# google/zopfli

Measured on AMD Instinct MI355X. Metric: input MB/s at numiterations=15 (gzip, bit-exact vs reference), higher is better.
Workload: dtype u8 (f32/f64 cost DP); 1 GPU; class-T synthetic (text-like, the enwik8 stand-in) 100000000 B per GPU, numiterations=15, blocksplitting=0, gzip, BASELINE configs[1]; total_bytes=100000000, master_blocks=100, gather=none (one rank)

## Files before the change

include/zopfli_amd.h:

```cpp
#ifndef ZOPFLI_AMD_H_
#define ZOPFLI_AMD_H_

#include <stddef.h>
#include <stdint.h>

#ifdef __cplusplus
extern "C" {
#endif

#if defined(__GNUC__)
#pragma GCC visibility push(default)
#endif



typedef struct ZopfliOptions {
  int verbose;
  int verbose_more;
  int numiterations;
  int blocksplitting;
  int blocksplittinglast;
  int blocksplittingmax;
} ZopfliOptions;

// ... 172 lines not shown
int zmx_last_host_timing(double* out2);

int zmx_last_match_timing(double* out4);
int zmx_last_match_walk(double* out3);

typedef void (*zmx_oom_hook_t)(int device);
void zmx_set_oom_hook(zmx_oom_hook_t hook);
int zmx_ctx_set_share(zmx_ctx* ctx, unsigned contexts_on_device);
int zmx_ctx_trim_cache(zmx_ctx* ctx);
int zmx_ctx_set_priority(zmx_ctx* ctx, int level);

int zmx_set_match_kernel(int kernel);

int zmx_last_seg_stats(double* out8);

#if defined(__GNUC__)
#pragma GCC visibility pop
#endif

#ifdef __cplusplus
}
#endif

#endif
```

zopfli_amd/api.py:

```python
import ctypes
import os

from ._build import LIB

if os.environ.get("ZOPFLI_AMD_LIB"):
    LIB = os.environ["ZOPFLI_AMD_LIB"]

FORMAT_GZIP, FORMAT_ZLIB, FORMAT_DEFLATE = 0, 1, 2
CRC32, ADLER32 = 0, 1
ZMX_HIST = 320


class ZopfliOptions(ctypes.Structure):
    _fields_ = [("verbose", ctypes.c_int), ("verbose_more", ctypes.c_int), ("numiterations", ctypes.c_int),
                ("blocksplitting", ctypes.c_int), ("blocksplittinglast", ctypes.c_int),
                ("blocksplittingmax", ctypes.c_int)]

    def __init__(self, numiterations=15, blocksplitting=1, blocksplittingmax=15, verbose=0, verbose_more=0):
        super().__init__(verbose, verbose_more, numiterations, blocksplitting, 0, blocksplittingmax)


class ZmxBlock(ctypes.Structure):
    _fields_ = [("instart", ctypes.c_uint64), ("inend", ctypes.c_uint64)]

# ... 63 lines not shown
                                    P(ctypes.c_uint32), P(ctypes.c_uint32)]
    lib.zmx_store_download.argtypes = [vp, vp, sz, ctypes.c_int, P(ctypes.c_uint16), P(ctypes.c_uint16), sz]
    lib.zmx_find_longest_match.argtypes = [vp, vp, sz, sz, P(ctypes.c_uint16), P(ctypes.c_uint16),
                                           P(ctypes.c_uint16)]
    lib.zmx_length_array_download.argtypes = [vp, vp, sz, P(ctypes.c_uint16)]
    lib.zmx_hash_links_download.argtypes = [vp, vp, sz, P(ctypes.c_uint16), P(ctypes.c_uint16), P(ctypes.c_uint16)]
    lib.zmx_deflate_range.argtypes = [vp, opt, sz, sz, ctypes.c_int, P(_u8p), P(sz)]
    lib.zmx_checksum.argtypes = [vp, ctypes.c_int, sz, sz, P(ctypes.c_uint32)]
    lib.zmx_checksum_combine.argtypes = [ctypes.c_int, ctypes.c_uint32, ctypes.c_uint32, ctypes.c_uint64]
    lib.zmx_checksum_combine.restype = ctypes.c_uint32
    lib.zmx_chunks_merge.argtypes = [P(vp), P(sz), sz, P(ctypes.c_ubyte), P(_u8p), P(sz)]
    lib.zmx_last_timing.argtypes = [P(ctypes.c_double)]
    lib.zmx_last_kernel_timing.argtypes = [P(ctypes.c_double)]
    lib.zmx_last_host_timing.argtypes = [P(ctypes.c_double)]
    lib.zmx_last_seg_stats.argtypes = [P(ctypes.c_double)]
    lib.zmx_last_match_timing.argtypes = [P(ctypes.c_double)]
    lib.zmx_set_match_kernel.argtypes = [ctypes.c_int]
    lib.zmx_dist_unique_id.argtypes = [ctypes.c_char_p]
    lib.zmx_dist_init.argtypes = [vp, ctypes.c_int, ctypes.c_int, ctypes.c_char_p, P(vp)]
    lib.zmx_dist_destroy.argtypes = [vp]
    lib.zmx_dist_destroy.restype = None
    lib.zmx_dist_comm_count.argtypes = [vp]
    lib.zmx_dist_gather.argtypes = [vp, vp, sz, P(vp), P(sz)]
    lib.zmx_set_kernel_timing.argtypes = [ctypes.c_int]
    lib.zmx_set_kernel_timing.restype = None
    lib.zmx_set_kernel_timing(1)
    return lib


def library(path=None):
# ... 73 lines not shown
    m = (ctypes.c_double * 4)()
    lib.zmx_last_match_timing(m)
    d["match_kernel"], d["hash_kernels"], d["table_builds"], d["positions_matched"] = m[0], m[1], m[2], m[3]
    w = (ctypes.c_double * 3)()
    lib.zmx_last_match_walk(w)
    d["skip_walk_lane_iterations"], d["skip_walk_wave_iterations"], d["skip_walk_positions"] = w[0], w[1], w[2]
    return d


def last_seg_stats(lib=None):
    lib = lib or library()
    t = (ctypes.c_double * 8)()
    lib.zmx_last_seg_stats(t)
    keys = ["tasks", "accepted", "rerun_state", "rerun_level", "rerun_tie", "positions_rerun", "rerun_values", "positions"]
    return dict(zip(keys, list(t)))


class Context:

    def __init__(self, device=0, lib=None):
        self.lib = lib or library()
        self.handle = ctypes.c_void_p()
        self._input = None
        self._segments = None
        if self.lib.zmx_ctx_create(device, ctypes.byref(self.handle)) != 0:
            raise RuntimeError("zmx_ctx_create: " + self.error())

    def error(self):
        return (self.lib.zmx_last_error() or b"").decode()

# ... 326 lines not shown
```

zopfli_amd/csrc/device/zmx_hip.hip:

```cpp
#include <hip/hip_runtime.h>

#include <algorithm>
#include <atomic>
#include <cmath>
#include <cstdio>
#include <cstdlib>
#include <cstring>
#include <mutex>
#include <string>
#include <unordered_map>
#include <vector>

#include "zmx_kernels.h"
#include "zmx_match2.h"
#ifdef ZMX_EXPERIMENTS
#include "zmx_match3.h"
#include "zmx_match4.h"
#else
#define BK_CH 32768u
#endif
#include "zmx_match5.h"
#include "zmx_dp4.h"
#include "zmx_dp5.h"
#include "zmx_encode.h"
// ... 4 lines not shown
#include "zmx_png_brute.h"
#include "zmx_blockcost.h"
#include "zopfli_amd.h"
#include "../host/symbol_check.h"
#include "../host/thread_pool.h"

namespace {

thread_local std::string g_err;
struct ThreadStats {
  double kernel_seconds[3];
  double squeeze_launches;
  double match5[3];
  double match[4];
  double seg[8];
};
static_assert(sizeof(ThreadStats) == 19 * sizeof(double), "zmx_internal_stats_take / _add move 19 doubles");
thread_local ThreadStats g_ts = {};
#define g_kernel_seconds g_ts.kernel_seconds
#define g_squeeze_launches g_ts.squeeze_launches
#define g_match5_stats g_ts.match5
#define g_match_stats g_ts.match
#define g_seg_stats g_ts.seg

thread_local bool g_last_oom = false;
thread_local int g_err_class = ZMX_ERR_NONE;

int Fail(const char* what, hipError_t e, const char* file, int line) {
  char buf[512];
  std::snprintf(buf, sizeof(buf), "%s: %s (%s:%d)", what, hipGetErrorString(e), file, line);
  g_err = buf;
  g_last_oom = e == hipErrorOutOfMemory;
  g_err_class = g_last_oom ? ZMX_ERR_OUT_OF_MEMORY : ZMX_ERR_DEVICE;
  if (g_last_oom) (void)hipGetLastError();
  return -1;
}
int FailMsg(const std::string& m) {
  g_err = m;
// ... 110 lines not shown
  double* d_cost = nullptr;
  double* d_mincost = nullptr;
  int* d_slot = nullptr;
  uint2* d_dph = nullptr;
  u64* d_block_edges = nullptr;
  u32* d_badpos = nullptr;
  size_t badpos_words = 0;
  bool badpos_clean = false;
  u64* d_code_base = nullptr;
  u16* d_codes = nullptr;
  double* d_wtab = nullptr;
  u32* d_badcodes = nullptr;
  u32* d_seg_off = nullptr;
  u32* d_extab = nullptr;
  uint2* d_seginfo = nullptr;
  std::vector<u32> seg_off;
  std::vector<u64> block_edges;
  std::vector<u32> tile_off;
  u32* d_counters = nullptr;
  u32* d_flags = nullptr;
  unsigned char* d_runin = nullptr;
  unsigned char* d_runout = nullptr;
  unsigned char* h_runin = nullptr;
  unsigned char* h_runout = nullptr;
  size_t h_runin_cap = 0, h_runout_cap = 0;
  size_t runin_bytes = 0, runout_bytes = 0;
  u64* d_prof = nullptr;
  std::vector<SegTask> tasks;
  std::vector<u32> task_off;
  SegTask* d_tasks = nullptr;
// ... 268 lines not shown
  if (kernel != 0 && kernel != 2 && kernel != 5) return FailMsg("zmx_set_match_kernel: 0, 2 or 5");
#endif
  g_match_kernel.store(kernel, std::memory_order_relaxed);
  return 0;
}

size_t zmx_internal_input_size(zmx_ctx* ctx) { return ctx->insize; }
int zmx_internal_device(zmx_ctx* ctx) { return ctx->device; }
void zmx_internal_set_error(const char* msg) { g_err = msg; g_err_class = ZMX_ERR_DEVICE; }
void zmx_internal_set_error_class(const char* msg, int cls) { g_err = msg; g_err_class = cls; }
const unsigned char* zmx_internal_input_host(zmx_ctx* ctx) { return ctx->h_in; }

void zmx_internal_seg_stats(double* out8, int reset) {
  for (int i = 0; i < 8; ++i) out8[i] = g_seg_stats[i];
  if (reset) for (int i = 0; i < 8; ++i) g_seg_stats[i] = 0;
}

void zmx_internal_match5_stats(double* out3, int reset) {
  for (int i = 0; i < 3; ++i) out3[i] = g_match5_stats[i];
  if (reset) for (int i = 0; i < 3; ++i) g_match5_stats[i] = 0;
}

void zmx_internal_match_stats(double* out4, int reset) {
  for (int i = 0; i < 4; ++i) out4[i] = g_match_stats[i];
  if (reset) for (int i = 0; i < 4; ++i) g_match_stats[i] = 0;
}

void zmx_internal_kernel_stats(double* seconds3, double* squeeze_launches, int reset) {
  for (int i = 0; i < 3; ++i) seconds3[i] = g_kernel_seconds[i];
  *squeeze_launches = g_squeeze_launches;
  if (reset) {
    g_kernel_seconds[0] = g_kernel_seconds[1] = g_kernel_seconds[2] = 0;
    g_squeeze_launches = 0;
  }
}

void zmx_internal_stats_take(double* out19) {
  std::memcpy(out19, &g_ts, sizeof(g_ts));
  g_ts = ThreadStats{};
}
void zmx_internal_stats_add(const double* in19) {
  double* d = reinterpret_cast<double*>(&g_ts);
  for (int i = 0; i < 19; ++i) d[i] += in19[i];
}

static hipError_t PinnedTake(zmx_ctx* c, unsigned char** p, size_t bytes, size_t* cap) {
  size_t best = c->pinned_free.size();
  for (size_t i = 0; i < c->pinned_free.size(); ++i) {
    const size_t k = c->pinned_free[i].second;
    if (k >= bytes && k <= 4 * bytes + 4096 && (best == c->pinned_free.size() || k < c->pinned_free[best].second)) best = i;
  }
  if (best != c->pinned_free.size()) {
    *p = c->pinned_free[best].first;
    *cap = c->pinned_free[best].second;
    c->pinned_free.erase(c->pinned_free.begin() + static_cast<long>(best));
    return hipSuccess;
  }
  *cap = bytes < 4096 ? 4096 : bytes;
// ... 21 lines not shown
  c->device = device;
  HIPCHK(hipStreamCreate(&c->stream));
  for (int i = 0; i < 4; ++i) HIPCHK(hipEventCreate(&c->ev[i]));
  HIPCHK(hipStreamCreate(&c->stream2));
  for (int i = 0; i < 2; ++i) HIPCHK(hipEventCreateWithFlags(&c->ev2[i], hipEventDisableTiming));
  {
    size_t mem_free = 0, mem_total = 0;
    HIPCHK(hipMemGetInfo(&mem_free, &mem_total));
    c->keep_base = std::min<size_t>(kPoolKeepMax, mem_free / 3);
    c->pool_keep = c->keep_base;
    c->code_budget = c->keep_base;
  }

  HIPCHK(hipFuncSetAttribute(reinterpret_cast<const void*>(k_chain), hipFuncAttributeMaxDynamicSharedMemorySize,
                             CH_LDS_BYTES));
#ifdef ZMX_EXPERIMENTS
  HIPCHK(hipFuncSetAttribute(reinterpret_cast<const void*>(k_bucket), hipFuncAttributeMaxDynamicSharedMemorySize,
                             BK_LDS_BYTES));
#endif
  *out = c;
  return 0;
}

int zmx_ctx_set_priority(zmx_ctx* c, int level) {
  DeviceGuard dev_guard(c->device);
  HIPCHK(dev_guard.err);
  const int k = level > 0 ? 1 : level < 0 ? 2 : 0;
  if (!c->alt_stream[0][0]) { c->alt_stream[0][0] = c->stream; c->alt_stream[0][1] = c->stream2; }
  if (k && !c->alt_stream[k][1]) {
    int least = 0, greatest = 0;
// ... 70 lines not shown
  rel(t->d_ssame);
  rel(t->d_chunk_base);
  rel(t->d_recs);
  rel(t->d_pool);
  rel(t->d_la);
  rel(t->d_dph);
  rel(t->d_block_edges);
  rel(t->d_badpos);
  rel(t->d_code_base);
  rel(t->d_codes);
  rel(t->d_wtab);
  rel(t->d_badcodes);
  rel(t->d_seg_off);
  rel(t->d_extab);
  rel(t->d_seginfo);
  rel(t->d_counters);
  rel(t->d_prof);
  rel(t->d_tasks);
  rel(t->d_task_off);
  rel(t->d_wg_tasks);
  rel(t->d_task_kind);
  rel(t->d_run_list);
  rel(t->d_wmeta);
  rel(t->d_runin);
  rel(t->d_runout);
  rel(t->d_winroff);
  rel(t->d_winflag);
  rel(t->d_win_off);
  rel(t->d_lvl);
  rel(t->d_entry);
// ... 151 lines not shown
  } else
#endif
  {
    HIPCHK(PoolAlloc(c, &t->d_links, reg_off));
  }
  HIPCHK(PoolAlloc(c, &t->d_recs, pos_off * 8));
  HIPCHK(PoolAlloc(c, &t->d_la, la_off));
  HIPCHK(PoolAlloc(c, &t->d_store[0], pos_off));
  HIPCHK(PoolAlloc(c, &t->d_store[1], pos_off));
  {
    const size_t in_cost = 0, in_min = in_cost + nb * ZMX_HIST * sizeof(double), in_info = in_min + nb * sizeof(double),
                 in_slot = in_info + 3 * nb * sizeof(float);
    t->runin_bytes = in_slot + nb * sizeof(int);
    const size_t out_hist = 0, out_nsym = out_hist + nb * ZMX_HIST * sizeof(u32), out_stats = out_nsym + nb * sizeof(u32),
                 out_flags = out_stats + 8 * sizeof(u32);
    t->runout_bytes = out_flags + 4 * sizeof(u32);
    HIPCHK(PoolAlloc(c, &t->d_runin, t->runin_bytes));
    HIPCHK(PoolAlloc(c, &t->d_runout, t->runout_bytes));
    HIPCHK(PinnedTake(c, &t->h_runin, t->runin_bytes, &t->h_runin_cap));
    HIPCHK(PinnedTake(c, &t->h_runout, t->runout_bytes, &t->h_runout_cap));
    t->d_cost = reinterpret_cast<double*>(t->d_runin + in_cost);
    t->d_mincost = reinterpret_cast<double*>(t->d_runin + in_min);
    t->d_runinfo = reinterpret_cast<float*>(t->d_runin + in_info);
    t->d_slot = reinterpret_cast<int*>(t->d_runin + in_slot);
    t->d_hist = reinterpret_cast<u32*>(t->d_runout + out_hist);
    t->d_nsym = reinterpret_cast<u32*>(t->d_runout + out_nsym);
    t->d_segstats = reinterpret_cast<u32*>(t->d_runout + out_stats);
    t->d_flags = reinterpret_cast<u32*>(t->d_runout + out_flags);
    HIPCHK(hipMemsetAsync(t->d_segstats, 0, 12 * sizeof(u32), c->stream));
  }
  HIPCHK(PoolAlloc(c, &t->d_dph, pos_off));
  HIPCHK(PoolAlloc(c, &t->d_block_edges, nb));
  t->badpos_words = pos_off / 32 + 4;
  HIPCHK(PoolAlloc(c, &t->d_badpos, t->badpos_words));
  HIPCHK(PoolAlloc(c, &t->d_code_base, nb));
  HIPCHK(PoolAlloc(c, &t->d_wtab, nb * ZMX_WTAB));
  HIPCHK(PoolAlloc(c, &t->d_badcodes, nb * 40));
  HIPCHK(PoolAlloc(c, &t->d_counters, 48));
  HIPCHK(hipMemcpyAsync(t->d_blocks, t->blocks.data(), nb * sizeof(BlockDesc), hipMemcpyHostToDevice, c->stream));
  HIPCHK(hipMemcpyAsync(t->d_tile_off, tile_off.data(), (nb + 1) * sizeof(u32), hipMemcpyHostToDevice, c->stream));
  HIPCHK(hipMemsetAsync(t->d_flags, 0, 4 * sizeof(u32), c->stream));

  HIPCHK(hipEventRecord(c->ev[0], c->stream));
  PoolScope hash_tmp(c);
  u16* d_lev = nullptr;
  u16* d_tot2 = nullptr;
  u16* d_rank2 = nullptr;
  uint4* d_xrec = nullptr;
  u32* d_tot12 = nullptr;
  unsigned long long* d_energy = nullptr;
  u32* d_cmax = nullptr;
  bool skip_any = false, skip_all = false;
  double skip_positions = 0;
  unsigned long long* d_m5stats = nullptr;
  bool join_stream2 = false;
  auto launch_hash = [&](const u64* d_link_lo) -> int {
    if (max_l == 0) return 0;
    const dim3 g1(static_cast<unsigned>((max_l + 256 * SAME_CH - 1) / (256 * SAME_CH)), static_cast<unsigned>(nb));
    hipLaunchKernelGGL(k_same, g1, dim3(256), 0, c->stream, c->d_in, t->d_blocks, t->d_same16, d_link_lo);
    KCHK(c, "k_same");
    HIPCHK(hipGetLastError());
    const dim3 g2(static_cast<unsigned>((max_l + CH_EMIT - 1) / CH_EMIT), static_cast<unsigned>(nb), 2);
#ifdef ZMX_EXPERIMENTS
    if (t->buckets) {
      BucketParams kp;
      kp.in = c->d_in;
      kp.blocks = t->d_blocks;
      kp.same16 = t->d_same16;
      kp.chunk_base = t->d_chunk_base;
      kp.link_lo = d_link_lo;
      for (int h = 0; h < 2; ++h) { kp.sorted[h] = t->d_sorted[h]; kp.rank[h] = t->d_rank[h]; kp.bucket[h] = t->d_bucket[h]; }
      kp.ssame = t->d_ssame;
      hipLaunchKernelGGL(k_bucket, g2, dim3(BK_THREADS), BK_LDS_BYTES, c->stream, kp);
      KCHK(c, "k_bucket");
    } else
#endif
    {
      hipLaunchKernelGGL(k_chain, g2, dim3(64), CH_LDS_BYTES, c->stream, c->d_in, t->d_blocks, t->d_same16, t->d_links, d_link_lo);
      KCHK(c, "k_chain");
      if ((mk == 5 || mk == 0) && d_link_lo == nullptr) {
        skip_any = mk == 5;
        if (mk == 5) for (size_t b = 0; b < nb; ++b) skip_positions += static_cast<double>(t->blocks[b].inend - t->blocks[b].instart);
        const unsigned hits_chunks = static_cast<unsigned>((max_l + RK_CH - 1) / RK_CH);
        {
          static const bool rank_all = [] { const char* e = std::getenv("ZOPFLI_AMD_RANK_ALL"); return e && std::atoi(e) != 0; }();
          if (!d_energy) HIPCHK(hash_tmp.AllocT(&d_energy, nb, "d_energy"));
          if (!d_cmax && !rank_all) HIPCHK(hash_tmp.AllocT(&d_cmax, nb * static_cast<size_t>(hits_chunks) + 1, "d_cmax"));
          HIPCHK(hipMemsetAsync(d_energy, 0, nb * sizeof(unsigned long long), c->stream));
          if (d_cmax) HIPCHK(hipMemsetAsync(d_cmax, 0, (nb * static_cast<size_t>(hits_chunks) + 1) * sizeof(u32), c->stream));
          HitsParams hp;
          hp.in = c->d_in;
          hp.blocks = t->d_blocks;
          hp.same16 = t->d_same16;
          hp.energy = d_energy;
// ... 481 lines not shown
      if (ntk) HIPCHK(hipMemcpyAsync(t->d_task_kind, kind.data(), ntk * sizeof(u32), hipMemcpyHostToDevice, c->stream));
      if (!runs.empty()) HIPCHK(hipMemcpyAsync(t->d_run_list, runs.data(), runs.size() * sizeof(u32), hipMemcpyHostToDevice, c->stream));
      HIPCHK(hipStreamSynchronize(c->stream));
    }
    wg.insert(wg.end(), wg_runs.begin(), wg_runs.end());
    HIPCHK(PoolAlloc(c, &t->d_wg_tasks, wg.size() + 4));
    if (!wg.empty()) HIPCHK(hipMemcpyAsync(t->d_wg_tasks, wg.data(), wg.size() * sizeof(u32), hipMemcpyHostToDevice, c->stream));
    HIPCHK(hipStreamSynchronize(c->stream));
  }
  }
  t->seg_off.assign(nb + 1, 0);
  for (size_t b = 0; b < nb; ++b) t->seg_off[b + 1] = t->seg_off[b] + (t->bsize[b] + TS_SEG - 1) / TS_SEG;
  HIPCHK(PoolAlloc(c, &t->d_seg_off, nb + 1));
  HIPCHK(PoolAlloc(c, &t->d_extab, static_cast<size_t>(t->seg_off[nb]) * GS_STATES));
  HIPCHK(PoolAlloc(c, &t->d_seginfo, t->seg_off[nb]));
  HIPCHK(hipMemcpyAsync(t->d_seg_off, t->seg_off.data(), (nb + 1) * sizeof(u32), hipMemcpyHostToDevice, c->stream));
  HIPCHK(hipStreamSynchronize(c->stream));
  return 0;
}

int zmx_tables_build(zmx_ctx* c, const zmx_block* blocks, size_t nblocks, zmx_tables** out) {
  return zmx_tables_build_from(c, nullptr, blocks, nblocks, out);
}

int zmx_tables_build_matches(zmx_ctx* c, const zmx_block* blocks, size_t nblocks, zmx_tables** out) {
  DeviceGuard dev_guard(c->device);
  HIPCHK(dev_guard.err);
  zmx_tables* t = new zmx_tables();
  g_last_oom = false;
  const int rc = BuildTables(c, blocks, nblocks, t, nullptr, false);
// ... 230 lines not shown
  tp.seg_off = t->d_seg_off;
  tp.nb_total = static_cast<u32>(nb);
  tp.recs = t->d_recs;
  tp.pool = t->d_pool;
  tp.la = t->d_la;
  tp.slot = t->d_slot;
  tp.store0 = t->d_store[0];
  tp.store1 = t->d_store[1];
  tp.hist_out = t->d_hist;
  tp.nsym_out = t->d_nsym;
  tp.flags = t->d_flags;
  tp.extab = t->d_extab;
  tp.seginfo = t->d_seginfo;
  tp.block0 = 0;
  tp.seg0 = 0;
  double ksec[3] = {0, 0, 0};
  const bool timing = KernelTiming();
  const dim3 dpdim(64 * (D3_NB + 2));
  {
    const unsigned nblk = static_cast<unsigned>(nb);
    const unsigned tiles = t->tile_off[nb];
    const unsigned ntask = t->task_off[nb];
    if (timing) HIPCHK(hipEventRecord(c->ev[0], c->stream));
    hipLaunchKernelGGL(k_wtab, dim3(nblk), dim3(256), 0, c->stream, wp);
    KCHK(c, "k_wtab");
    if (tiles && scan_bad) hipLaunchKernelGGL(k_badscan, dim3(tiles), dim3(256), 0, c->stream, bp);
    KCHK(c, "k_badscan");
    HIPCHK(hipGetLastError());
    if (timing) HIPCHK(hipEventRecord(c->ev[1], c->stream));
    {
// ... 46 lines not shown
        } else {
          if (cp.prof) hipLaunchKernelGGL((k_dp5_spec<true, 4, false>), dim3(cap), dim3(64 * D5_WG), 0, c->stream, c2);
          else hipLaunchKernelGGL((k_dp5_spec<false, 4, false>), dim3(cap), dim3(64 * D5_WG), 0, c->stream, c2);
        }
        KCHK(c, "k_dp5_spec");
        hipLaunchKernelGGL(k_dpcheck, dim3(ntask), dim3(64), 0, c->stream, cp);
        KCHK(c, "k_dpcheck");
      }
      if (cp.prof) hipLaunchKernelGGL(k_dp4_fix<true>, dim3(nblk), dpdim, 0, c->stream, cp);
      else hipLaunchKernelGGL(k_dp4_fix<false>, dim3(nblk), dpdim, 0, c->stream, cp);
      KCHK(c, "k_dp4_fix");
    }
    HIPCHK(hipGetLastError());
    if (timing) HIPCHK(hipEventRecord(c->ev[2], c->stream));
    const unsigned nseg = t->seg_off[nb];
    if (nseg) hipLaunchKernelGGL(k_trace_exits, dim3(nseg), dim3(TS_THREADS), 0, c->stream, tp);
    KCHK(c, "k_trace_exits");
    hipLaunchKernelGGL(k_trace_link, dim3(nblk), dim3(64), 0, c->stream, tp);
    KCHK(c, "k_trace_link");
    if (nseg) hipLaunchKernelGGL(k_trace_emit, dim3(nseg), dim3(64), 0, c->stream, tp);
    KCHK(c, "k_trace_emit");
    HIPCHK(hipGetLastError());
    if (timing) HIPCHK(hipEventRecord(c->ev[3], c->stream));
  }
  u32 segstats[8];
  HIPCHK(hipMemcpyAsync(t->h_runout, t->d_runout, t->runout_bytes, hipMemcpyDeviceToHost, c->stream));
  HIPCHK(hipStreamSynchronize(c->stream));
  for (int i = 0; i < 3 && timing; ++i) {
    float ms = 0;
    HIPCHK(hipEventElapsedTime(&ms, c->ev[i], c->ev[i + 1]));
    ksec[i] += ms * 1e-3;
  }
  {
    const u32* o_hist = reinterpret_cast<const u32*>(t->h_runout);
    const u32* o_nsym = o_hist + nb * ZMX_HIST;
    const u32* o_stats = o_nsym + nb;
    const u32* o_flags = o_stats + 8;
    std::memcpy(hist, o_hist, nb * ZMX_HIST * sizeof(u32));
    std::memcpy(nsym, o_nsym, nb * sizeof(u32));
    std::memcpy(segstats, o_stats, sizeof(segstats));
    if (o_flags[1]) {
      char buf[128];
      std::snprintf(buf, sizeof(buf), "zmx_squeeze_run: device consistency flags 0x%x", o_flags[1]);
      return FailFault(buf);
    }
  }
  t->h_hist.assign(hist, hist + nb * ZMX_HIST);
  t->have_hist = true;
  ++t->squeeze_runs;
  {
    for (int i = 0; i < 3; ++i) g_kernel_seconds[i] += ksec[i];
    g_squeeze_launches += 1;
// ... 817 lines not shown
```

zopfli_amd/csrc/device/zmx_kernels.h:

```cpp
#pragma once
#include <hip/hip_runtime.h>
#include <stdint.h>

typedef unsigned char u8;
typedef unsigned short u16;
typedef unsigned int u32;
typedef unsigned long long u64;

struct BlockDesc {
  u64 instart, inend, ws;
  u64 pos_off;
  u64 reg_off;
  u64 la_off;
};

#define ZMX_WINDOW 32768u
#define ZMX_MAX_MATCH 258u
#define ZMX_MAX_CHAIN_HITS 8192
#define ZMX_NONE16 0xffffu

__device__ __forceinline__ int dev_dist_symbol(u32 d) {
  if (d < 5) return (int)d - 1;
  const int l = 31 - __clz((int)(d - 1));
  return 2 * l + (int)(((d - 1) >> (l - 1)) & 1);
// ... 170 lines not shown
      u32 d;
      if (lower) d = lane - (63u - (u32)__clzll((long long)lower));
      else d = old == ZMX_NONE16 ? 0u : r - old;
      if (d > 32767u) d = 0;
      wave_lds_sync();
      if (act && (grp & gt_mask) == 0) head[key] = (u16)r;
      wave_lds_sync();
      const u64 k = t0 + i;
      if (act && k >= e0) {
        if (chain == 0) {
          lk[k].x = (u16)d;
          lk[k].z = sames[i];
        } else {
          lk[k].y = (u16)d;
        }
      }
    }
    __syncthreads();
  }
}

#define MT 2048u
#define MWIN_BYTES (32768u + MT + 288u)
#define SCRATCH_CPS 256u
#define M_XCD_GROUP 16u
#define MATCH_BATCH 8u

struct MatchParams {
  const u8* in;
  const BlockDesc* blocks;
// ... 384 lines not shown
```

zopfli_amd/csrc/device/zmx_trace.h:

```cpp
#pragma once

#define TS_SEG 4096u
#define TS_ENT 258u

struct TraceSegParams {
  const BlockDesc* blocks;
  const u32* seg_off;
  u32 nb_total;
  u32 block0;
  u32 seg0;
  const u32* recs;
  const u32* pool;
  const u16* la;
  const int* slot;
  u32* store0;
  u32* store1;
  u32* hist_out;
  u32* nsym_out;
  u32* flags;
  u32* extab;
  uint2* seginfo;
};

__device__ __forceinline__ void ts_bounds(u32 B, u32 s, u32& lo, u32& hi) {
  hi = B - s * TS_SEG;
  lo = hi > TS_SEG ? hi - TS_SEG : 0u;
}

__device__ __forceinline__ u32 ts_find_block(const u32* seg_off, u32 nb, u32 seg) {
  u32 lo = 0, hi = nb;
  while (hi - lo > 1) {
    const u32 mid = (lo + hi) >> 1;
    if (seg_off[mid] <= seg) lo = mid; else hi = mid;
  }
  return lo;
}

#define TS_ROUNDS 6
#define TS_THREADS 512u

__global__ __launch_bounds__(TS_THREADS) void k_trace_exits(TraceSegParams P) {
  __shared__ u32 s_j[TS_SEG + 1];
  const u32 seg = P.seg0 + blockIdx.x;
  const u32 b = ts_find_block(P.seg_off, P.nb_total, seg);
  const BlockDesc bd = P.blocks[b];
  const u32 B = (u32)(bd.inend - bd.instart);
  u32 lo, hi;
  ts_bounds(B, seg - P.seg_off[b], lo, hi);
  const u16* la = P.la + bd.la_off;
  const u32 n = hi - lo;
  for (u32 x = threadIdx.x + 1; x <= n; x += TS_THREADS) {
    const u32 h = lo + x;
    u32 len = la[h];
    if (len == 0) len = 1;
    if (len > h) len = h;
    const u32 t = h - len;
    s_j[x] = (t > lo ? t - lo : 0x8000u | (lo - t)) | (1u << 16);
  }
// ... 13 lines not shown
    u32 v = s_j[n - j];
    while (!(v & 0x8000u)) {
      const u32 w = s_j[v & 0xffffu];
      v = (w & 0xffffu) | ((v & 0xffff0000u) + (w & 0xffff0000u));
    }
    P.extab[(u64)seg * TS_ENT + j] = (v & 0x7fffu) | (v & 0xffff0000u);
  }
}

__global__ __launch_bounds__(64) void k_trace_link(TraceSegParams P) {
  const u32 b = P.block0 + blockIdx.x;
  const BlockDesc bd = P.blocks[b];
  const u32 B = (u32)(bd.inend - bd.instart);
  const u32 lane = threadIdx.x;
  for (u32 i = lane; i < 320; i += 64) P.hist_out[(u64)b * 320 + i] = 0;
  if (lane != 0) return;
  const u32 s0 = P.seg_off[b], ns = P.seg_off[b + 1] - s0;
  u32 j = 0, off = 0;
  for (u32 s = 0; s < ns; ++s) {
    P.seginfo[s0 + s] = make_uint2(j, off);
    u32 lo, hi;
    ts_bounds(B, s, lo, hi);
    if (hi - lo <= j) {
      P.seginfo[s0 + s] = make_uint2(0xffffffffu, off);
      continue;
    }
    const u32 v = P.extab[(u64)(s0 + s) * TS_ENT + j];
    off += v >> 16;
    j = v & 0xffffu;
  }
  P.nsym_out[b] = off;
}
// ... 137 lines not shown
```

zopfli_amd/csrc/host/api.cc:

```cpp
#include <chrono>
#include <malloc.h>
#include <cstdio>
#include <cstdlib>
#include <cstring>
#include <algorithm>
#include <condition_variable>
#include <memory>
#include <mutex>
#include <string>
#include <thread>
#include <unordered_map>
#include <vector>

#include "block_cache.h"
#include "block_cost.h"
#include "deflate.h"
#include "lz77_optimal.h"
#include "symbols.h"
#include "deal.h"
#include "dealing.h"
#include "thread_pool.h"
#include "zopfli_amd.h"

extern "C" void zmx_internal_kernel_stats(double* seconds3, double* squeeze_launches, int reset);
extern "C" void zmx_internal_seg_stats(double* out8, int reset);
extern "C" void zmx_internal_match_stats(double* out4, int reset);
extern "C" void zmx_internal_match5_stats(double* out3, int reset);
extern "C" void zmx_internal_stats_take(double* out19);
extern "C" void zmx_internal_stats_add(const double* in19);
extern "C" size_t zmx_internal_input_size(zmx_ctx* ctx);
extern "C" const unsigned char* zmx_internal_input_host(zmx_ctx* ctx);
extern "C" void zmx_internal_set_error(const char* msg);

namespace {

using zamd::kMasterBlock;

[[noreturn]] void Die(const char* what) {
  std::fprintf(stderr, "zopfli_amd: %s: %s\n", what, zmx_last_error());
  std::exit(EXIT_FAILURE);
}

void MaybeKeepHeap() {
  static const bool once = [] {
// ... 309 lines not shown
    ~InlineHostWork() { if (on) zamd::g_host_inline = was; }
  } inline_host(parts.size() <= 2 && Pool().InFlight() > 1);
  const std::vector<zmx_ctx*>& ctxs = lease.ctxs;
  const size_t ndev = std::min(ctxs.size(), parts.size());
  struct Shard {
    size_t first = 0, last = 0, base = 0;
    std::vector<zamd::Chunk> chunks;
    std::vector<size_t> part_chunks;
    int rc = 0;
    std::string err;
    int err_class = ZMX_ERR_NONE;
    zamd::Timing timing;
    uint32_t sum = 0;
    size_t sum_bytes = 0;
    bool redone = false;
    double stats[19] = {0};
  };
  std::vector<Shard> shards(ndev);
  for (size_t d = 0; d < ndev; ++d) {
    shards[d].first = parts.size() * d / ndev;
    shards[d].last = parts.size() * (d + 1) / ndev;
  }
  static const bool deal_by_cost = [] { const char* e = std::getenv("ZOPFLI_AMD_DEAL"); return !e || std::strcmp(e, "count") != 0; }();
  if (deal_by_cost && ndev > 1 && in != nullptr && parts.size() > ndev) {
    std::vector<double> cost(parts.size());
    zamd::ParallelFor(parts.size(), [&](size_t i) { cost[i] = zamd::MasterBlockCost(in, parts[i].instart, parts[i].inend); });
    std::vector<size_t> first;
    zamd::DealByCost(cost, ndev, &first);
    for (size_t d = 0; d < ndev; ++d) { shards[d].first = first[d]; shards[d].last = first[d + 1]; }
  }
  if (const char* e = std::getenv("ZOPFLI_AMD_SHARD_WEIGHTS")) {
// ... 411 lines not shown
int zmx_last_match_timing(double* out4) {
  zmx_internal_match_stats(out4, 0);
  return 0;
}

int zmx_last_match_walk(double* out3) {
  zmx_internal_match5_stats(out3, 0);
  return 0;
}

int zmx_last_seg_stats(double* out8) {
  zmx_internal_seg_stats(out8, 0);
  return 0;
}

int zmx_last_host_timing(double* out2) {
  out2[0] = zamd::ThreadTiming().download;
  out2[1] = zamd::ThreadTiming().serialize;
  return 0;
}

namespace {
zamd::Histogram RangeHistogram(const ZopfliLZ77Store* lz77, size_t lstart, size_t lend) {
  zamd::Histogram h;
  h.Clear();
  for (size_t i = lstart; i < lend; ++i) {
    if (lz77->dists[i] == 0) {
      h.ll[lz77->litlens[i]]++;
    } else {
      h.ll[zamd::LengthSymbol(lz77->litlens[i])]++;
// ... 38 lines not shown
```

Before: 799.9 MB/s.

## Fuse hash-chain build into single-pass kernel and add funnel fast path for trace exits

Replaces the default k_same + k_chain pair with a new k_hash kernel. It computes run lengths, both hash keys and chain links in one pass, using per-wave LDS head tables and an optional long-emit mode with periodic head aging. It also adds a k_trace_funnel pre-pass: when a segment's exit paths converge within a bounded depth, it resolves the segment's exit table with one wave via a prefix-max scan and pointer jumping. Only unresolved segments fall back to the 512-thread k_trace_exits. A host-side statistic turns the funnel off adaptively when most segments get listed, at the cost of an extra launch and considerably more kernel complexity.

```diff
diff --git a/include/zopfli_amd.h b/include/zopfli_amd.h
--- a/include/zopfli_amd.h
+++ b/include/zopfli_amd.h
@@ -210,6 +210,8 @@
 
 int zmx_last_seg_stats(double* out8);
 
+int zmx_last_trace_stats(double* out2);
+
 #if defined(__GNUC__)
 #pragma GCC visibility pop
 #endif
diff --git a/zopfli_amd/api.py b/zopfli_amd/api.py
--- a/zopfli_amd/api.py
+++ b/zopfli_amd/api.py
@@ -101,6 +101,7 @@
     lib.zmx_last_kernel_timing.argtypes = [P(ctypes.c_double)]
     lib.zmx_last_host_timing.argtypes = [P(ctypes.c_double)]
     lib.zmx_last_seg_stats.argtypes = [P(ctypes.c_double)]
+    lib.zmx_last_trace_stats.argtypes = [P(ctypes.c_double)]
     lib.zmx_last_match_timing.argtypes = [P(ctypes.c_double)]
     lib.zmx_set_match_kernel.argtypes = [ctypes.c_int]
     lib.zmx_dist_unique_id.argtypes = [ctypes.c_char_p]
@@ -204,6 +205,13 @@
     lib.zmx_last_seg_stats(t)
     keys = ["tasks", "accepted", "rerun_state", "rerun_level", "rerun_tie", "positions_rerun", "rerun_values", "positions"]
     return dict(zip(keys, list(t)))
+
+
+def last_trace_stats(lib=None):
+    lib = lib or library()
+    t = (ctypes.c_double * 2)()
+    lib.zmx_last_trace_stats(t)
+    return {"segments": t[0], "listed": t[1]}
 
 
 class Context:
diff --git a/zopfli_amd/csrc/device/zmx_hip.hip b/zopfli_amd/csrc/device/zmx_hip.hip
--- a/zopfli_amd/csrc/device/zmx_hip.hip
+++ b/zopfli_amd/csrc/device/zmx_hip.hip
@@ -42,14 +42,16 @@
   double match5[3];
   double match[4];
   double seg[8];
+  double trace[2];
 };
-static_assert(sizeof(ThreadStats) == 19 * sizeof(double), "zmx_internal_stats_take / _add move 19 doubles");
+static_assert(sizeof(ThreadStats) == 21 * sizeof(double), "zmx_internal_stats_take / _add move 21 doubles");
 thread_local ThreadStats g_ts = {};
 #define g_kernel_seconds g_ts.kernel_seconds
 #define g_squeeze_launches g_ts.squeeze_launches
 #define g_match5_stats g_ts.match5
 #define g_match_stats g_ts.match
 #define g_seg_stats g_ts.seg
+#define g_trace_stats g_ts.trace
 
 thread_local bool g_last_oom = false;
 thread_local int g_err_class = ZMX_ERR_NONE;
@@ -190,6 +192,9 @@
   u32* d_seg_off = nullptr;
   u32* d_extab = nullptr;
   uint2* d_seginfo = nullptr;
+  u32* d_fblist = nullptr;
+  u32* d_tstat = nullptr;
+  bool funnel_off = false;
   std::vector<u32> seg_off;
   std::vector<u64> block_edges;
   std::vector<u32> tile_off;
@@ -488,7 +493,9 @@
 void zmx_internal_seg_stats(double* out8, int reset) {
   for (int i = 0; i < 8; ++i) out8[i] = g_seg_stats[i];
   if (reset) for (int i = 0; i < 8; ++i) g_seg_stats[i] = 0;
-}
+  if (reset) g_trace_stats[0] = g_trace_stats[1] = 0;
+}
+
 
 void zmx_internal_match5_stats(double* out3, int reset) {
   for (int i = 0; i < 3; ++i) out3[i] = g_match5_stats[i];
@@ -509,13 +516,13 @@
   }
 }
 
-void zmx_internal_stats_take(double* out19) {
-  std::memcpy(out19, &g_ts, sizeof(g_ts));
+void zmx_internal_stats_take(double* out21) {
+  std::memcpy(out21, &g_ts, sizeof(g_ts));
   g_ts = ThreadStats{};
 }
-void zmx_internal_stats_add(const double* in19) {
+void zmx_internal_stats_add(const double* in21) {
   double* d = reinterpret_cast<double*>(&g_ts);
-  for (int i = 0; i < 19; ++i) d[i] += in19[i];
+  for (int i = 0; i < 21; ++i) d[i] += in21[i];
 }
 
 static hipError_t PinnedTake(zmx_ctx* c, unsigned char** p, size_t bytes, size_t* cap) {
@@ -567,6 +574,10 @@
 
   HIPCHK(hipFuncSetAttribute(reinterpret_cast<const void*>(k_chain), hipFuncAttributeMaxDynamicSharedMemorySize,
                              CH_LDS_BYTES));
+  HIPCHK(hipFuncSetAttribute(reinterpret_cast<const void*>(k_hash<false>), hipFuncAttributeMaxDynamicSharedMemorySize,
+                             HF_LDS_BYTES));
+  HIPCHK(hipFuncSetAttribute(reinterpret_cast<const void*>(k_hash<true>), hipFuncAttributeMaxDynamicSharedMemorySize,
+                             HF_LDS_BYTES));
 #ifdef ZMX_EXPERIMENTS
   HIPCHK(hipFuncSetAttribute(reinterpret_cast<const void*>(k_bucket), hipFuncAttributeMaxDynamicSharedMemorySize,
                              BK_LDS_BYTES));
@@ -667,6 +678,7 @@
   rel(t->d_seg_off);
   rel(t->d_extab);
   rel(t->d_seginfo);
+  rel(t->d_fblist);
   rel(t->d_counters);
   rel(t->d_prof);
   rel(t->d_tasks);
@@ -848,7 +860,8 @@
     t->runin_bytes = in_slot + nb * sizeof(int);
     const size_t out_hist = 0, out_nsym = out_hist + nb * ZMX_HIST * sizeof(u32), out_stats = out_nsym + nb * sizeof(u32),
                  out_flags = out_stats + 8 * sizeof(u32);
-    t->runout_bytes = out_flags + 4 * sizeof(u32);
+    const size_t out_tstat = out_flags + 4 * sizeof(u32);
+    t->runout_bytes = out_tstat + 2 * sizeof(u32);
     HIPCHK(PoolAlloc(c, &t->d_runin, t->runin_bytes));
     HIPCHK(PoolAlloc(c, &t->d_runout, t->runout_bytes));
     HIPCHK(PinnedTake(c, &t->h_runin, t->runin_bytes, &t->h_runin_cap));
@@ -861,7 +874,8 @@
     t->d_nsym = reinterpret_cast<u32*>(t->d_runout + out_nsym);
     t->d_segstats = reinterpret_cast<u32*>(t->d_runout + out_stats);
     t->d_flags = reinterpret_cast<u32*>(t->d_runout + out_flags);
-    HIPCHK(hipMemsetAsync(t->d_segstats, 0, 12 * sizeof(u32), c->stream));
+    t->d_tstat = reinterpret_cast<u32*>(t->d_runout + out_tstat);
+    HIPCHK(hipMemsetAsync(t->d_segstats, 0, 14 * sizeof(u32), c->stream));
   }
   HIPCHK(PoolAlloc(c, &t->d_dph, pos_off));
   HIPCHK(PoolAlloc(c, &t->d_block_edges, nb));
@@ -890,10 +904,14 @@
   bool join_stream2 = false;
   auto launch_hash = [&](const u64* d_link_lo) -> int {
     if (max_l == 0) return 0;
-    const dim3 g1(static_cast<unsigned>((max_l + 256 * SAME_CH - 1) / (256 * SAME_CH)), static_cast<unsigned>(nb));
-    hipLaunchKernelGGL(k_same, g1, dim3(256), 0, c->stream, c->d_in, t->d_blocks, t->d_same16, d_link_lo);
-    KCHK(c, "k_same");
-    HIPCHK(hipGetLastError());
+    const char* hash_env = std::getenv("ZOPFLI_AMD_HASH");
+    const bool hash_pair = hash_env && std::strcmp(hash_env, "pair") == 0;
+    if (hash_pair || t->buckets) {
+      const dim3 g1(static_cast<unsigned>((max_l + 256 * SAME_CH - 1) / (256 * SAME_CH)), static_cast<unsigned>(nb));
+      hipLaunchKernelGGL(k_same, g1, dim3(256), 0, c->stream, c->d_in, t->d_blocks, t->d_same16, d_link_lo);
+      KCHK(c, "k_same");
+      HIPCHK(hipGetLastError());
+    }
     const dim3 g2(static_cast<unsigned>((max_l + CH_EMIT - 1) / CH_EMIT), static_cast<unsigned>(nb), 2);
 #ifdef ZMX_EXPERIMENTS
     if (t->buckets) {
@@ -910,8 +928,18 @@
     } else
 #endif
     {
-      hipLaunchKernelGGL(k_chain, g2, dim3(64), CH_LDS_BYTES, c->stream, c->d_in, t->d_blocks, t->d_same16, t->d_links, d_link_lo);
-      KCHK(c, "k_chain");
+      if (hash_pair) {
+        hipLaunchKernelGGL(k_chain, g2, dim3(64), CH_LDS_BYTES, c->stream, c->d_in, t->d_blocks, t->d_same16, t->d_links, d_link_lo);
+        KCHK(c, "k_chain");
+      } else {
+        const char* emit_env = std::getenv("ZOPFLI_AMD_HASH_EMIT");
+        u32 emit = emit_env ? static_cast<u32>(std::atoi(emit_env)) : HF_EMIT_DEFAULT;
+        if (emit != 65536u && emit != 131072u) emit = CH_EMIT;
+        const dim3 gh(static_cast<unsigned>((max_l + emit - 1) / emit), static_cast<unsigned>(nb));
+        if (emit == CH_EMIT) hipLaunchKernelGGL(k_hash<false>, gh, dim3(128), HF_LDS_BYTES, c->stream, c->d_in, t->d_blocks, t->d_same16, t->d_links, d_link_lo, emit);
+        else hipLaunchKernelGGL(k_hash<true>, gh, dim3(128), HF_LDS_BYTES, c->stream, c->d_in, t->d_blocks, t->d_same16, t->d_links, d_link_lo, emit);
+        KCHK(c, "k_hash");
+      }
       if ((mk == 5 || mk == 0) && d_link_lo == nullptr) {
         skip_any = mk == 5;
         if (mk == 5) for (size_t b = 0; b < nb; ++b) skip_positions += static_cast<double>(t->blocks[b].inend - t->blocks[b].instart);
@@ -1423,6 +1451,7 @@
   HIPCHK(PoolAlloc(c, &t->d_seg_off, nb + 1));
   HIPCHK(PoolAlloc(c, &t->d_extab, static_cast<size_t>(t->seg_off[nb]) * GS_STATES));
   HIPCHK(PoolAlloc(c, &t->d_seginfo, t->seg_off[nb]));
+  HIPCHK(PoolAlloc(c, &t->d_fblist, static_cast<size_t>(t->seg_off[nb]) + 1));
   HIPCHK(hipMemcpyAsync(t->d_seg_off, t->seg_off.data(), (nb + 1) * sizeof(u32), hipMemcpyHostToDevice, c->stream));
   HIPCHK(hipStreamSynchronize(c->stream));
   return 0;
@@ -1683,6 +1712,18 @@
   tp.seginfo = t->d_seginfo;
   tp.block0 = 0;
   tp.seg0 = 0;
+  tp.nseg = t->seg_off[nb];
+  tp.fb_list = t->d_fblist;
+  tp.tstat = t->d_tstat;
+  {
+    const char* e_on = std::getenv("ZOPFLI_AMD_FUNNEL");
+    const char* e_depth = std::getenv("ZOPFLI_AMD_FUNNEL_DEPTH");
+    const int mode = e_on ? std::atoi(e_on) : 1;
+    int depth = e_depth ? std::atoi(e_depth) : static_cast<int>(TF_DEPTH_MAX);
+    if (depth > static_cast<int>(TF_DEPTH_MAX)) depth = TF_DEPTH_MAX;
+    if (depth < static_cast<int>(TS_ENT) || mode == 0 || (mode != 2 && t->funnel_off)) depth = 0;
+    tp.funnel_depth = static_cast<u32>(depth);
+  }
   double ksec[3] = {0, 0, 0};
   const bool timing = KernelTiming();
   const dim3 dpdim(64 * (D3_NB + 2));
@@ -1759,6 +1800,10 @@
     HIPCHK(hipGetLastError());
     if (timing) HIPCHK(hipEventRecord(c->ev[2], c->stream));
     const unsigned nseg = t->seg_off[nb];
+    if (nseg && tp.funnel_depth) {
+      hipLaunchKernelGGL(k_trace_funnel, dim3((nseg + TF_WAVES - 1) / TF_WAVES), dim3(64 * TF_WAVES), 0, c->stream, tp);
+      KCHK(c, "k_trace_funnel");
+    }
     if (nseg) hipLaunchKernelGGL(k_trace_exits, dim3(nseg), dim3(TS_THREADS), 0, c->stream, tp);
     KCHK(c, "k_trace_exits");
     hipLaunchKernelGGL(k_trace_link, dim3(nblk), dim3(64), 0, c->stream, tp);
@@ -1781,6 +1826,10 @@
     const u32* o_nsym = o_hist + nb * ZMX_HIST;
     const u32* o_stats = o_nsym + nb;
     const u32* o_flags = o_stats + 8;
+    const u32* o_tstat = o_flags + 4;
+    g_trace_stats[0] += o_tstat[0];
+    g_trace_stats[1] += o_tstat[1];
+    if (tp.funnel_depth && 2ull * o_tstat[1] > o_tstat[0]) t->funnel_off = true;
     std::memcpy(hist, o_hist, nb * ZMX_HIST * sizeof(u32));
     std::memcpy(nsym, o_nsym, nb * sizeof(u32));
     std::memcpy(segstats, o_stats, sizeof(segstats));
diff --git a/zopfli_amd/csrc/device/zmx_kernels.h b/zopfli_amd/csrc/device/zmx_kernels.h
--- a/zopfli_amd/csrc/device/zmx_kernels.h
+++ b/zopfli_amd/csrc/device/zmx_kernels.h
@@ -208,6 +208,218 @@
         } else {
           lk[k].y = (u16)d;
         }
+      }
+    }
+    __syncthreads();
+  }
+}
+
+#define HF_TILE 2048u
+#define HF_HALF 1024u
+#define HF_EMIT_DEFAULT 65536u
+#define HF_LDS_BYTES (2 * 65536 + HF_TILE * 6)
+
+__device__ __forceinline__ uint4 ld16_unaligned(const u8* p) {
+  uint4 v;
+  __builtin_memcpy(&v, p, 16);
+  return v;
+}
+__device__ __forceinline__ u32 first_other_byte(uint4 v, u32 c) {
+  const u32 pat = c * 0x01010101u;
+  const u32 w[4] = {v.x ^ pat, v.y ^ pat, v.z ^ pat, v.w ^ pat};
+  u32 r = 16;
+#pragma unroll
+  for (int i = 3; i >= 0; --i) {
+    if (w[i]) r = 4u * i + ((u32)(__ffs((int)w[i]) - 1) >> 3);
+  }
+  return r;
+}
+
+template <bool LONG>
+__global__ __launch_bounds__(128) void k_hash(const u8* __restrict__ in, const BlockDesc* __restrict__ blocks,
+                                              u16* __restrict__ same16, ushort4* __restrict__ links,
+                                              const u64* __restrict__ link_lo, u32 emit) {
+  extern __shared__ __align__(16) u8 dyn_lds[];
+  u16* head_all = reinterpret_cast<u16*>(dyn_lds);
+  u16* keys_all = head_all + 65536;
+  u16* sames = keys_all + 2 * HF_TILE;
+
+  const BlockDesc bd = blocks[blockIdx.y];
+  const u64 L = bd.inend - bd.ws;
+  const u64 e0 = (u64)blockIdx.x * emit;
+  if (e0 >= L) return;
+  const u64 e1 = (e0 + emit < L) ? e0 + emit : L;
+  if (link_lo && e1 <= link_lo[blockIdx.y]) return;
+  const u64 w0 = e0 >= ZMX_WINDOW ? e0 - ZMX_WINDOW : 0;
+  const u32 wave = (u32)__builtin_amdgcn_readfirstlane((int)(threadIdx.x >> 6));
+  const u32 lane = threadIdx.x & 63u;
+  const u64 lt_mask = (1ull << lane) - 1;
+  const u64 gt_mask = ~((2ull << lane) - 1);
+  u16* head = head_all + 32768u * wave;
+  u16* keys = keys_all + HF_TILE * wave;
+
+  {
+    const u32 none = LONG ? 0x80008000u : ~0u;
+    for (u32 i = lane; i < 4096; i += 64) reinterpret_cast<uint4*>(head)[i] = make_uint4(none, none, none, none);
+  }
+
+  const u8* base = in + bd.ws;
+  u16* same = same16 + bd.reg_off;
+  ushort4* lk = links + bd.reg_off;
+  u64 run_end = 0;
+  bool run_have = false, run_done = false;
+  __syncthreads();
+
+  for (u64 t0 = w0; t0 < e1; t0 += HF_TILE) {
+    const u32 tn = (u32)((e1 - t0 < HF_TILE) ? e1 - t0 : HF_TILE);
+    const u32 hoff = HF_HALF * wave;
+    const u32 hn = tn > hoff ? (tn - hoff < HF_HALF ? tn - hoff : HF_HALF) : 0u;
+    if (hn) {
+      const u64 h0 = t0 + hoff;
+      const u32 i0 = 16u * lane;
+      const bool lane_on = i0 < hn;
+      u32 by[18];
+      {
+        uint4 v = make_uint4(0, 0, 0, 0);
+        u32 b16 = 0, b17 = 0;
+        if (lane_on) {
+          const u8* p = base + h0 + i0;
+          v = ld16_unaligned(p);
+          b16 = p[16];
+          b17 = p[17];
+        }
+        const u64 left = lane_on ? L - (h0 + i0) : 0;
+        const u32 nv = left < 18 ? (u32)left : 18u;
+        const u32 w[4] = {v.x, v.y, v.z, v.w};
+#pragma unroll
+        for (u32 q = 0; q < 16; ++q) by[q] = q < nv ? (w[q >> 2] >> (8u * (q & 3u))) & 255u : 0u;
+        by[16] = 16 < nv ? b16 : 0u;
+        by[17] = 17 < nv ? b17 : 0u;
+        u32 stops = 0;
+#pragma unroll
+        for (u32 q = 0; q < 16; ++q) stops |= (q + 1 < nv && by[q + 1] == by[q]) ? 0u : 1u << q;
+        u64 end_abs = 0;
+        const bool need = hn == HF_HALF && !((rdlane_u32(stops, 63) >> 15) & 1u);
+        if (need) {
+          const u64 pl = h0 + HF_HALF - 1;
+          const u32 c = rdlane_u32(by[15], 63);
+          const u64 limit = pl + 65535u < L - 1 ? pl + 65535u : L - 1;
+          if (!(run_have && run_end >= pl)) { run_end = pl; run_done = false; run_have = true; }
+          while (!run_done && run_end < limit) {
+            const u64 pos = run_end + 1 + 16u * lane;
+            u32 mm = 0;
+            if (pos < L) {
+              mm = first_other_byte(ld16_unaligned(base + pos), c);
+              if (L - pos < mm) mm = (u32)(L - pos);
+            }
+            const u64 other = __ballot(mm < 16u);
+            if (other) {
+              const u32 fl = (u32)__ffsll((long long)other) - 1u;
+              run_end += 16u * fl + rdlane_u32(mm, fl);
+              run_done = true;
+            } else {
+              run_end += 1024u;
+            }
+          }
+          if (!run_done && run_end >= L - 1) { run_end = L - 1; run_done = true; }
+          end_abs = run_end;
+        }
+        const u64 with_stop = __ballot(stops != 0u);
+        const u64 above = with_stop & gt_mask;
+        const u32 my_first = i0 + (u32)(__ffs((int)stops) - 1);
+        const u32 src = above ? (u32)__ffsll((long long)above) - 1u : lane;
+        const u32 from_above = (u32)__shfl((int)my_first, (int)src);
+        const u64 far = end_abs > h0 ? end_abs - h0 : 0;
+        u32 end_rel = above ? from_above : (far < (1u << 20) ? (u32)far : 1u << 20);
+        u32 sm[16];
+#pragma unroll
+        for (int q = 15; q >= 0; --q) {
+          if ((stops >> q) & 1u) end_rel = i0 + (u32)q;
+          const u32 s = end_rel - (i0 + (u32)q);
+          sm[q] = s < 65535u ? s : 65535u;
+        }
+        if (lane_on) {
+          u32 k0[8], k1[8], sp[8];
+#pragma unroll
+          for (u32 q = 0; q < 16; q += 2) {
+            const u32 va = ((by[q] << 10) ^ (by[q + 1] << 5) ^ by[q + 2]) & 32767u;
+            const u32 vb = ((by[q + 1] << 10) ^ (by[q + 2] << 5) ^ by[q + 3]) & 32767u;
+            k0[q >> 1] = va | (vb << 16);
+            k1[q >> 1] = (va ^ ((sm[q] - 3u) & 255u)) | ((vb ^ ((sm[q + 1] - 3u) & 255u)) << 16);
+            sp[q >> 1] = sm[q] | (sm[q + 1] << 16);
+          }
+          uint4* d0 = reinterpret_cast<uint4*>(keys_all + hoff + i0);
+          uint4* d1 = reinterpret_cast<uint4*>(keys_all + HF_TILE + hoff + i0);
+          uint4* ds = reinterpret_cast<uint4*>(sames + hoff + i0);
+          d0[0] = make_uint4(k0[0], k0[1], k0[2], k0[3]); d0[1] = make_uint4(k0[4], k0[5], k0[6], k0[7]);
+          d1[0] = make_uint4(k1[0], k1[1], k1[2], k1[3]); d1[1] = make_uint4(k1[4], k1[5], k1[6], k1[7]);
+          ds[0] = make_uint4(sp[0], sp[1], sp[2], sp[3]); ds[1] = make_uint4(sp[4], sp[5], sp[6], sp[7]);
+        }
+      }
+    }
+    __syncthreads();
+    const u32 cur0 = (u32)(t0 - w0);
+    const bool warm = t0 < e0;
+    if (LONG && cur0 != 0 && (cur0 & 16383u) == 0) {
+      const u32 now = (cur0 & 0xffffu) * 0x00010001u, stale = now ^ 0x80008000u;
+      for (u32 i = lane; i < 4096; i += 64) {
+        uint4 h = reinterpret_cast<uint4*>(head)[i];
+        u32 hw[4] = {h.x, h.y, h.z, h.w};
+#pragma unroll
+        for (int k = 0; k < 4; ++k) {
+          const u32 lo_age = ((now & 0xffffu) - (hw[k] & 0xffffu)) & 0x8000u;
+          const u32 hi_age = ((now >> 16) - (hw[k] >> 16)) & 0x8000u;
+          const u32 m = (lo_age ? 0xffffu : 0u) | (hi_age ? 0xffff0000u : 0u);
+          hw[k] = (hw[k] & ~m) | (stale & m);
+        }
+        reinterpret_cast<uint4*>(head)[i] = make_uint4(hw[0], hw[1], hw[2], hw[3]);
+      }
+      wave_lds_sync();
+    }
+    for (u32 i0 = 0; i0 < tn; i0 += 64) {
+      const u32 i = i0 + lane;
+      const bool act = i < tn;
+      const u32 key = act ? (u32)keys[i] : 0u;
+      const u32 r = cur0 + i;
+      if (warm) {
+        bool todo = act;
+        while (__any(todo)) {
+          if (todo) head[key] = (u16)r;
+          wave_lds_sync();
+          const u32 w = act ? (u32)head[key] : 0xffffu;
+          wave_lds_sync();
+          todo = act && (LONG ? ((r - w) & 0xffffu) - 1u < 63u : w < r);
+        }
+        continue;
+      }
+      const u32 old = act ? (u32)head[key] : (LONG ? (r ^ 0x8000u) & 0xffffu : (u32)ZMX_NONE16);
+      u64 grp = __ballot(act);
+#pragma unroll
+      for (int bit = 0; bit < 15; ++bit) {
+        const bool mine = (key >> bit) & 1;
+        const u64 bm = __ballot(mine);
+        grp &= mine ? bm : ~bm;
+      }
+      const u64 lower = grp & lt_mask;
+      u32 d;
+      if (lower) d = lane - (63u - (u32)__clzll((long long)lower));
+      else if (LONG) d = (r - old) & 0xffffu;
+      else d = old == ZMX_NONE16 ? 0u : r - old;
+      if (d > 32767u) d = 0;
+      wave_lds_sync();
+      if (act) {
+        if ((grp & gt_mask) == 0) head[key] = (u16)r;
+        keys[i] = (u16)d;
+      }
+      wave_lds_sync();
+    }
+    __syncthreads();
+    if (!warm && hn) {
+      for (u32 j = lane; j < hn; j += 64) {
+        const u32 i = hoff + j;
+        const u16 s = sames[i];
+        lk[t0 + i] = make_ushort4(keys_all[i], keys_all[HF_TILE + i], s, 0);
+        same[t0 + i] = s;
       }
     }
     __syncthreads();
diff --git a/zopfli_amd/csrc/device/zmx_trace.h b/zopfli_amd/csrc/device/zmx_trace.h
--- a/zopfli_amd/csrc/device/zmx_trace.h
+++ b/zopfli_amd/csrc/device/zmx_trace.h
@@ -20,6 +20,10 @@
   u32* flags;
   u32* extab;
   uint2* seginfo;
+  u32 nseg;
+  u32 funnel_depth;
+  u32* fb_list;
+  u32* tstat;
 };
 
 __device__ __forceinline__ void ts_bounds(u32 B, u32 s, u32& lo, u32& hi) {
@@ -39,9 +43,149 @@
 #define TS_ROUNDS 6
 #define TS_THREADS 512u
 
+#define TF_WAVES 2u
+#define TF_DEPTH_MAX 1024u
+#define TF_WIN (TS_SEG / 64u)
+
+__global__ __launch_bounds__(64 * TF_WAVES) void k_trace_funnel(TraceSegParams P) {
+  __shared__ __align__(16) u16 s_cells[TF_WAVES][TS_SEG + 16];
+  static_assert((TF_DEPTH_MAX + 64) * sizeof(u32) <= (TS_SEG + 16) * sizeof(u16), "the jumps fit the cells' room");
+  const u32 wave = (u32)__builtin_amdgcn_readfirstlane((int)(threadIdx.x >> 6));
+  const u32 lane = threadIdx.x & 63u;
+  const u32 seg_i = blockIdx.x * TF_WAVES + wave;
+  if (seg_i >= P.nseg) return;
+  const u32 seg = P.seg0 + seg_i;
+  const u32 b = ts_find_block(P.seg_off, P.nb_total, seg);
+  const BlockDesc bd = P.blocks[b];
+  const u32 B = (u32)(bd.inend - bd.instart);
+  u32 lo, hi;
+  ts_bounds(B, seg - P.seg_off[b], lo, hi);
+  const u32 n = hi - lo;
+  bool listed = n < TS_ENT + 1 || P.funnel_depth < TS_ENT;
+  u32 q = 0;
+  u32 v[TF_WIN];
+  u16* cells = s_cells[wave];
+  if (!listed) {
+    const u16* la = P.la + bd.la_off;
+    const u32 a0 = (lo + 1) & ~7u;
+    const u32 pieces = (hi - a0) / 8u + 1u;
+    const u32 shift8 = TS_SEG / 8u + 1u - pieces;
+    uint4 c8[9];
+#pragma unroll
+    for (u32 r = 0; r < 9; ++r) {
+      const u32 i = lane + 64u * r;
+      c8[r] = *reinterpret_cast<const uint4*>(la + a0 + 8u * (i < pieces ? i : pieces - 1u));
+    }
+#define TF_PIN(A) "+v"(c8[A].x), "+v"(c8[A].y), "+v"(c8[A].z), "+v"(c8[A].w)
+    asm volatile("" : TF_PIN(0), TF_PIN(1), TF_PIN(2), TF_PIN(3), TF_PIN(4));
+    asm volatile("" : TF_PIN(5), TF_PIN(6), TF_PIN(7), TF_PIN(8));
+#undef TF_PIN
+#pragma unroll
+    for (u32 r = 0; r < 9; ++r) {
+      const u32 i = lane + 64u * r;
+      if (i < pieces) reinterpret_cast<uint4*>(cells)[shift8 + i] = c8[r];
+    }
+    wave_lds_sync();
+    {
+      const u32 top = 8u * shift8 + hi - a0;
+      const u16* low = cells + (top - lane - 64u * (TF_WIN - 1u));
+#pragma unroll
+      for (u32 w = 0; w < TF_WIN; ++w) v[w] = low[64u * (TF_WIN - 1u - w)];
+    }
+    wave_lds_sync();
+#pragma unroll
+    for (u32 w = 0; w < TF_WIN; ++w) {
+      const u32 x = 64u * w + lane;
+      const u32 h = hi - x;
+      u32 len = v[w];
+      if (len == 0) len = 1;
+      if (len > h) len = h;
+      v[w] = x < n ? len : 1u;
+    }
+    const u32 depth = P.funnel_depth < TF_DEPTH_MAX ? P.funnel_depth : TF_DEPTH_MAX;
+    u32 carry = 0;
+    bool found = false;
+#pragma unroll
+    for (u32 w = 0; w < TF_DEPTH_MAX / 64u; ++w) {
+      if (!found && 64u * w < depth && 64u * w < n) {
+        const u32 x = 64u * w + lane;
+        u32 m = wave_scan_max(x + v[w]);
+        m = m > carry ? m : carry;
+        const u32 c = x + 1;
+        const u64 ok = __ballot(m == c && c >= TS_ENT - 1 && c < n && c <= depth);
+        if (ok) {
+          q = 64u * w + (u32)__ffsll((long long)ok);
+          found = true;
+        }
+        carry = rdlane_u32(m, 63);
+      }
+    }
+    listed = !found;
+  }
+  if (lane == 0) P.fb_list[seg_i] = listed ? 1u : 0u;
+  if (seg_i == 0 && lane == 0) P.tstat[1] = 0;
+  if (listed) return;
+  u32* J = reinterpret_cast<u32*>(cells);
+#pragma unroll
+  for (u32 w = 0; w < TF_DEPTH_MAX / 64u + 1; ++w) {
+    if (64u * w <= q) {
+      const u32 x = 64u * w + lane;
+      if (x < q) J[x] = (x + v[w]) | (1u << 16);
+      else if (x == q) J[x] = q;
+    }
+  }
+  wave_lds_sync();
+  for (;;) {
+    bool moving = false;
+    for (u32 x = lane; x < q; x += 64) {
+      const u32 a = J[x];
+      if ((a & 0xffffu) != q) {
+        const u32 t = J[a & 0xffffu];
+        J[x] = (t & 0xffffu) | ((a & 0xffff0000u) + (t & 0xffff0000u));
+        moving = moving || (t & 0xffffu) != q;
+      }
+    }
+    wave_lds_sync();
+    if (!__any(moving)) break;
+  }
+  u32 steps = 0;
+  int at = (int)q;
+#pragma unroll
+  for (u32 w = 0; w < TF_WIN; ++w) {
+    const int base = (int)(64u * w);
+    const int lim = __builtin_amdgcn_readfirstlane((int)(n - 64u * w < 64u ? n - 64u * w : 64u));
+    if (64u * w < n && at - base < lim) {
+      int idx = at - base;
+      const u64 lit = __ballot(v[w] == 1u);
+      do {
+        const u32 len = rdlane_u32(v[w], (u32)idx);
+        if (len == 1u) {
+          const u64 other = ~(lit >> idx);
+          int run = other ? __ffsll((long long)other) - 1 : 64;
+          if (run > lim - idx) run = lim - idx;
+          idx += run;
+          steps += (u32)run;
+        } else {
+          idx += (int)len;
+          ++steps;
+        }
+      } while (idx < lim);
+      at = base + idx;
+    }
+  }
+  const u32 code = (u32)at - n;
+  for (u32 j = lane; j < TS_ENT; j += 64) {
+    if (j < n) P.extab[(u64)seg * TS_ENT + j] = code | (((J[j] >> 16) + steps) << 16);
+  }
+}
+
 __global__ __launch_bounds__(TS_THREADS) void k_trace_exits(TraceSegParams P) {
   __shared__ u32 s_j[TS_SEG + 1];
-  const u32 seg = P.seg0 + blockIdx.x;
+  const u32 seg_i = blockIdx.x;
+  if (P.funnel_depth >= TS_ENT) {
+    if (!P.fb_list[seg_i]) return;
+  }
+  const u32 seg = P.seg0 + seg_i;
   const u32 b = ts_find_block(P.seg_off, P.nb_total, seg);
   const BlockDesc bd = P.blocks[b];
   const u32 B = (u32)(bd.inend - bd.instart);
@@ -85,8 +229,21 @@
   const u32 B = (u32)(bd.inend - bd.instart);
   const u32 lane = threadIdx.x;
   for (u32 i = lane; i < 320; i += 64) P.hist_out[(u64)b * 320 + i] = 0;
+  const u32 s0 = P.seg_off[b], ns = P.seg_off[b + 1] - s0;
+  {
+    const bool funnels = P.funnel_depth >= TS_ENT;
+    u32 mine = 0;
+    if (funnels) for (u32 s = lane; s < ns; s += 64) mine += P.fb_list[s0 - P.seg0 + s];
+    const u32 listed = rdlane_u32(wave_scan_add(mine), 63);
+    if (lane == 0) {
+      if (funnels && listed) atomicAdd(&P.tstat[1], listed);
+      if (blockIdx.x == 0) {
+        P.tstat[0] = P.nseg;
+        if (!funnels) P.tstat[1] = P.nseg;
+      }
+    }
+  }
   if (lane != 0) return;
-  const u32 s0 = P.seg_off[b], ns = P.seg_off[b + 1] - s0;
   u32 j = 0, off = 0;
   for (u32 s = 0; s < ns; ++s) {
     P.seginfo[s0 + s] = make_uint2(j, off);
diff --git a/zopfli_amd/csrc/host/api.cc b/zopfli_amd/csrc/host/api.cc
--- a/zopfli_amd/csrc/host/api.cc
+++ b/zopfli_amd/csrc/host/api.cc
@@ -26,8 +26,8 @@
 extern "C" void zmx_internal_seg_stats(double* out8, int reset);
 extern "C" void zmx_internal_match_stats(double* out4, int reset);
 extern "C" void zmx_internal_match5_stats(double* out3, int reset);
-extern "C" void zmx_internal_stats_take(double* out19);
-extern "C" void zmx_internal_stats_add(const double* in19);
+extern "C" void zmx_internal_stats_take(double* out21);
+extern "C" void zmx_internal_stats_add(const double* in21);
 extern "C" size_t zmx_internal_input_size(zmx_ctx* ctx);
 extern "C" const unsigned char* zmx_internal_input_host(zmx_ctx* ctx);
 extern "C" void zmx_internal_set_error(const char* msg);
@@ -367,7 +367,7 @@
     uint32_t sum = 0;
     size_t sum_bytes = 0;
     bool redone = false;
-    double stats[19] = {0};
+    double stats[21] = {0};
   };
   std::vector<Shard> shards(ndev);
   for (size_t d = 0; d < ndev; ++d) {
@@ -809,6 +809,15 @@
   return 0;
 }
 
+int zmx_last_trace_stats(double* out2) {
+  double s[21] = {0};
+  zmx_internal_stats_take(s);
+  zmx_internal_stats_add(s);
+  out2[0] = s[19];
+  out2[1] = s[20];
+  return 0;
+}
+
 int zmx_last_host_timing(double* out2) {
   out2[0] = zamd::ThreadTiming().download;
   out2[1] = zamd::ThreadTiming().serialize;
```

Result: faster. 829.4 MB/s, median of 4 (+3.7%).
